# DigitalPhonetics/Intrinsic-Subgraph-Generation-for-VQA

Measured on AMD Instinct MI355X. Metric: GQA questions/sec, higher is better.
Workload: dtype f32

## Files before the change

### intrinsic-subgraph-generation-for-vqa_amd/csrc/isg_layer_tile.hip

```cpp
#include "isg_f16x3.hpp"

#include "isg_diag.hpp"

#include <type_traits>

ISG_DIAG_BUFFER(g_dt_stamps)
#define DT_STAMP(i) ISG_DIAG_ADD(i)
#define TC_STAMP(i) ISG_DIAG_ADD(i)

namespace isg {

constexpr int TP_CH = 1024;

__device__ __forceinline__ void tile_plan_body(const int *__restrict__ ptr, const int *__restrict__ eptr, int B, int ncap, int ecap,
                                               int *__restrict__ tile_ptr, int *__restrict__ ntiles, int cap,
                                               int4 *__restrict__ tile_info, int4 *__restrict__ tile_heavy_first = nullptr) {
  __shared__ int s_jump[2][TP_CH];
  __shared__ int s_mark[TP_CH];
  __shared__ int s_ptr[TP_CH + 1], s_eptr[TP_CH + 1];
  __shared__ int s_wsum[TP_CH / 64];
  __shared__ int s_base;
  const int i = threadIdx.x, lane = i & 63, wave = i >> 6;
  if (i == 0) s_base = 0;
  __syncthreads();
// ... 65 lines not shown
  if (tile_info && tile_heavy_first) {
    constexpr int NB = 9;
    constexpr int NW = TP_CH / 64;
    __shared__ int s_cnt[NW][NB];
    __shared__ int s_start[NB];
    __syncthreads();
    const int T = min(s_base, cap);
    int mine[NB];
#pragma unroll
    for (int b = 0; b < NB; ++b) mine[b] = 0;
    for (int t0 = 0; t0 < T; t0 += TP_CH) {
      const int t = t0 + i;
      const int cls = t < T ? NB - 1 - min((tile_info[t].w + 31) >> 5, NB - 1) : -1;
#pragma unroll
      for (int b = 0; b < NB; ++b) mine[b] += __popcll(__ballot(cls == b));
    }
    if (lane == 0) {
#pragma unroll
      for (int b = 0; b < NB; ++b) s_cnt[wave][b] = mine[b];
    }
    __syncthreads();
    if (i == 0) {
      int run = 0;
      for (int b = 0; b < NB; ++b) {
        int c = 0;
        for (int w = 0; w < NW; ++w) c += s_cnt[w][b];
        s_start[b] = run;
        run += c;
      }
    }
    __syncthreads();
    for (int t0 = 0; t0 < T; t0 += TP_CH) {
      const int t = t0 + i;
      int4 d = make_int4(0, 0, 0, 0);
      if (t < T) d = tile_info[t];
      const int cls = t < T ? NB - 1 - min((d.w + 31) >> 5, NB - 1) : -1;
      int below = 0, wcnt[NB];
#pragma unroll
      for (int b = 0; b < NB; ++b) {
        const unsigned long long m = __ballot(cls == b);
        wcnt[b] = __popcll(m);
        if (cls == b) below = __popcll(m & ((1ull << lane) - 1ull));
      }
      if (lane == 0) {
#pragma unroll
        for (int b = 0; b < NB; ++b) s_cnt[wave][b] = wcnt[b];
      }
      __syncthreads();
      if (cls >= 0) {
        int at = s_start[cls] + below;
        for (int w = 0; w < wave; ++w) at += s_cnt[w][cls];
        tile_heavy_first[at] = d;
      }
      __syncthreads();
      if (i < NB) {
        int c = 0;
        for (int w = 0; w < NW; ++w) c += s_cnt[w][i];
        s_start[i] += c;
      }
      __syncthreads();
    }
  }
}

__global__ __launch_bounds__(TP_CH) void tile_plan_kernel(const int *__restrict__ ptr, const int *__restrict__ eptr, int B,
                                                          int ncap, int ecap, int *__restrict__ tile_ptr,
                                                          int *__restrict__ ntiles, int cap, int4 *__restrict__ tile_info,
                                                          int4 *__restrict__ tile_heavy_first) {
  tile_plan_body(ptr, eptr, B, ncap, ecap, tile_ptr, ntiles, cap, tile_info, tile_heavy_first);
}

constexpr int DT_ROWS = 64, DT_KC = 128, DT_K1 = 512, DT_MID = 256, DT_C = 128;
constexpr int DT_LDA = DT_KC + 8, DT_LDY = DT_MID + 8, DT_LDC = DT_C + 4;
constexpr int DT_KS1 = DT_K1 / 16, DT_KS2 = DT_MID / 16;
constexpr int DT_BUF_BYTES = 2 * 2 * DT_ROWS * DT_LDA * 2;
constexpr int DT_GPC = 128;
constexpr int DT_GST = 8;
constexpr int DT_SMEM_BYTES = DT_BUF_BYTES + (3 * 64 + 4 * 64 + 64 + 64 + 64 + 2 * DT_GST * DT_C + DT_GPC + 4) * 4;
static_assert(2 * DT_ROWS * DT_LDY * 2 <= DT_BUF_BYTES && DT_ROWS * DT_LDC * 4 + 2 * 32 * DT_C * 4 <= DT_BUF_BYTES, "aliases must fit");
static_assert(2 * DT_SMEM_BYTES <= 160 * 1024, "two workgroups per CU");
constexpr int DT_GROUP_MAX = 4;
constexpr int DT_LIVE_SMEM_BYTES = DT_SMEM_BYTES + (DT_ROWS + DT_GROUP_MAX * DT_ROWS / 4 + 8) * 4;
static_assert(2 * DT_LIVE_SMEM_BYTES <= 160 * 1024, "two workgroups per CU");

struct DtArgs {
  const float *a;
  const float *a_rowmax;
  const _Float16 *w1f;
  const float *w1_inv, *b1;
  const float *y_bound;
  const _Float16 *w2f;
  const float *w2_inv, *b2;
  const float *ins, *h;
  const float *gn_w, *gn_b, *gn_ms;
  const float *node_mask, *ins_next;
  float *h_out;
  float *xg_out, *xinv_out;
  _Float16 *xp_out;
  const int *ptr, *tile_ptr, *ntiles;
  const int4 *tile_info;
  const long long *batch;
  int N, lda, P, ldp;
  float eps, denom;
  const unsigned *row_dead;
  int group, max_tiles;
};

template <bool LIVE>
__global__ __launch_bounds__(256, 2) void mgat_dense_tail_kernel(DtArgs a) {
  extern __shared__ __attribute__((aligned(16))) unsigned char dt_smem[];
  typedef _Float16 (*BufA)[2][DT_ROWS][DT_LDA];
  typedef _Float16 (*BufY)[DT_ROWS][DT_LDY];
  typedef float (*BufC)[DT_LDC];
  BufA bufA = reinterpret_cast<BufA>(dt_smem);
  BufY sY = reinterpret_cast<BufY>(dt_smem);
  BufC sC = reinterpret_cast<BufC>(dt_smem);
  float *s_f = reinterpret_cast<float *>(dt_smem + DT_BUF_BYTES);
  float *s_inv1 = s_f, *s_scale2 = s_f + 64, *s_inv2 = s_f + 128, *s_rmax = s_f + 192, *s_a = s_f + 448;
  int *s_gid = reinterpret_cast<int *>(s_f + 512);
  float *s_mask = s_f + 576;
  float *s_ins = s_f + 640, *s_insn = s_f + 640 + DT_GST * DT_C;

  int *s_gp = reinterpret_cast<int *>(s_f + 2688);
  int *s_list = reinterpret_cast<int *>(s_f + 2820);
  unsigned char *s_cpos = reinterpret_cast<unsigned char *>(s_f + 2884);
  int *s_w = reinterpret_cast<int *>(s_f + 2948);

  int tid = threadIdx.x, lane = tid & 63;
  const int wave = __builtin_amdgcn_readfirstlane(tid >> 6);
  int fr = lane & 31, hh = lane >> 5, fk = hh * 8;
  int srow = tid >> 5, sc4 = tid & 31;
  int gi = tid >> 5, c4 = tid & 31;
  int voff = lane * 16;
  int t = blockIdx.x, r0 = 0, nrows = 0, g0 = 0, g1 = 0, ng = 0, L = 0, tb = 0, t0 = 0, gt = 1;
  bool grouped = false;
  if constexpr (!LIVE) {
    const int4 tinfo = a.tile_info[t];
    if (t >= *a.ntiles) return;
    r0 = tinfo.x;
    nrows = min(tinfo.y, DT_ROWS);
    if (nrows <= 0) return;
    L = nrows;
    g0 = a.tile_ptr[t], g1 = a.tile_ptr[t + 1];
    ng = g1 - g0;
  } else {
    t0 = blockIdx.x * a.group;
    int4 ti[DT_GROUP_MAX];
#pragma unroll
    for (int k = 0; k < DT_GROUP_MAX; ++k) ti[k] = a.tile_info[min(t0 + k, a.max_tiles - 1)];
    const int nt = *a.ntiles;
    if (t0 >= nt) return;
    gt = min(a.group, nt - t0);
    int bk[DT_GROUP_MAX + 1];
    bk[0] = 0;
#pragma unroll
    for (int k = 0; k < DT_GROUP_MAX; ++k) bk[k + 1] = bk[k] + (k < gt ? max(min(ti[k].y, DT_ROWS), 0) : 0);
    const int total = bk[DT_GROUP_MAX];
    if (total == 0) return;
    int gr = ti[0].x + tid;
#pragma unroll
    for (int k = 1; k < DT_GROUP_MAX; ++k)
      if (tid >= bk[k]) gr = ti[k].x + tid - bk[k];
    const bool has = tid < total;
    gr = min(max(gr, 0), a.N - 1);
    const bool dead = has && a.row_dead[gr] == 0x01010101u;
    const bool live = has && !dead;
    const unsigned long long lb = __ballot(live), db = __ballot(dead);
    if (lane == 0) {
      s_w[wave] = __popcll(lb);
      s_w[4 + wave] = db ? wave * 64 + (int)__builtin_ctzll(db) : 256;
    }
    __syncthreads();
    int before = 0, nlive = 0, fd = 256;
#pragma unroll
    for (int w = 0; w < 4; ++w) {
      const int c = s_w[w];
      if (w < wave) before += c;
      nlive += c;
      fd = min(fd, s_w[4 + w]);
    }
    nlive = __builtin_amdgcn_readfirstlane(nlive);
    fd = __builtin_amdgcn_readfirstlane(fd);
    const int Lg = nlive + (fd < 256 ? 1 : 0);
    grouped = Lg <= DT_ROWS;
    if (grouped) {
      L = Lg;
      const int pos = before + __popcll(lb & ((1ull << lane) - 1ull));
      if (live) { s_list[pos] = gr; s_cpos[tid] = (unsigned char)pos; }
      if (dead) s_cpos[tid] = (unsigned char)nlive;
      if (tid == fd) s_list[nlive] = gr;
    }
  }
  ISG_DIAG_BEGIN()
  hf32x4 rh[8];
  int h_gid = 0, h_gp = 0;
  float h_mask = 1.f;
  float4 h_ins = make_float4(0.f, 0.f, 0.f, 0.f), h_insn = make_float4(0.f, 0.f, 0.f, 0.f);

#define DT_ROW(row) (LIVE ? s_list[min(row, L - 1)] : min(r0 + min(row, nrows - 1), a.N - 1))
  auto x_proj = [&](auto ni_c) __attribute__((always_inline)) {
  constexpr int NI = decltype(ni_c)::value;
  constexpr int NU = 4 * NI;
  if constexpr (LIVE) __syncthreads();
#define DT_LOAD_CHUNK(c)                                                                                         \
  _Pragma("unroll") for (int u = 0; u < NU; ++u) {                                                               \
    const int row = srow + 8 * u;                                                                                \
    const int gr = DT_ROW(row);                                                                                  \
    { const hf32x4 t_ = __builtin_nontemporal_load(reinterpret_cast<const hf32x4 *>(a.a + (int64_t)gr * a.lda + (c) * DT_KC + sc4 * 4)); ra[u] = make_float4(t_[0], t_[1], t_[2], t_[3]); } \
  }
  float4 ra[NU];
  DT_LOAD_CHUNK(0)
  const int hrow = DT_ROW(tid);
  const float *rm = a.a_rowmax + (int64_t)hrow * a.ldp;
  float rmv[4];
#pragma unroll
  for (int p = 0; p < 4; ++p) rmv[p] = rm[min(p, a.P - 1)];
#define DT_TAIL_REQUEST(trow)                                                                                    \
  h_gid = (int)a.batch[trow];                                                                                    \
  if (a.node_mask) h_mask = a.node_mask[trow];                       \
  h_gp = a.ptr[g0 + min(tid, ng)];                                                                               \
  {                                                                                                              \
    const int gi_c = min(gi, max(min(ng, DT_GST) - 1, 0));                                                       \
    h_ins = *reinterpret_cast<const float4 *>(a.ins + (int64_t)(g0 + gi_c) * DT_C + c4 * 4);                     \
    if (a.ins_next) h_insn = *reinterpret_cast<const float4 *>(a.ins_next + (int64_t)(g0 + gi_c) * DT_C + c4 * 4); \
  }
  if constexpr (!LIVE) { DT_TAIL_REQUEST(hrow) }
  if (tid < DT_ROWS) {
    float mx = fmaxf(fmaxf(rmv[0], rmv[1]), fmaxf(rmv[2], rmv[3]));
    for (int p = 4; p < a.P; ++p) mx = fmaxf(mx, rm[p]);
    float s, inv;
    h3_scale(mx, s, inv);
    s_rmax[tid] = s;
    s_inv1[tid] = inv;
    h3_scale(fmaf(mx, a.y_bound[0], a.y_bound[1]), s, inv);
    s_scale2[tid] = s;
    s_inv2[tid] = inv;
    if constexpr (!LIVE) {
      s_gid[tid] = h_gid;
      s_mask[tid] = h_mask;
    }
  }
#define DT_TAIL_FILE()                                                                                           \
  if (tid <= min(ng, DT_GPC)) s_gp[tid] = h_gp - r0;                                                             \
  if (gi < min(ng, DT_GST)) {                                                                                    \
    *reinterpret_cast<float4 *>(&s_ins[gi * DT_C + c4 * 4]) = h_ins;                                             \
    if (a.ins_next) *reinterpret_cast<float4 *>(&s_insn[gi * DT_C + c4 * 4]) = h_insn;                           \
  }
  if constexpr (!LIVE) { DT_TAIL_FILE() }
  __syncthreads();
  float sa[NU];
#pragma unroll
  for (int u = 0; u < NU; ++u) sa[u] = s_rmax[srow + 8 * u];
#define DT_WRITE_CHUNK(b)                                                                                        \
  _Pragma("unroll") for (int u = 0; u < NU; ++u) {                                                               \
    const int row = srow + 8 * u;                                                                                \
    float4 v = ra[u];                                                                                            \
    if (row >= L) v = make_float4(0.f, 0.f, 0.f, 0.f);                                                           \
    v.x *= sa[u]; v.y *= sa[u]; v.z *= sa[u]; v.w *= sa[u];                                                      \
    hf16x4 hi = {(_Float16)v.x, (_Float16)v.y, (_Float16)v.z, (_Float16)v.w};                                    \
    hf16x4 mid = {(_Float16)(v.x - (float)hi[0]), (_Float16)(v.y - (float)hi[1]), (_Float16)(v.z - (float)hi[2]), \
                  (_Float16)(v.w - (float)hi[3])};                                                               \
    *reinterpret_cast<hf16x4 *>(&bufA[b][0][row][sc4 * 4]) = hi;                                                 \
    *reinterpret_cast<hf16x4 *>(&bufA[b][1][row][sc4 * 4]) = mid;                                                \
  }
  DT_STAMP(0)
  DT_WRITE_CHUNK(0)
  DT_LOAD_CHUNK(1)

  constexpr unsigned plane1 = (unsigned)(DT_MID / 32) * DT_KS1 * 1024u;
  const __amdgpu_buffer_rsrc_t wr1 =
      __builtin_amdgcn_make_buffer_rsrc(const_cast<_Float16 *>(a.w1f), 0, (int)(2u * plane1), 0x00020000);
  hf32x16 acc[NI][2];
#pragma unroll
  for (int i = 0; i < NI; ++i)
#pragma unroll
    for (int j = 0; j < 2; ++j)
#pragma unroll
      for (int r = 0; r < 16; ++r) acc[i][j][r] = 0.f;
  hf16x8 wq[4][2][2], af[NI][2];
#define DT_LOADW1(st, s)                                                                                         \
  _Pragma("unroll") for (int j = 0; j < 2; ++j) _Pragma("unroll") for (int q = 0; q < 2; ++q)                    \
      wq[st][j][q] = __builtin_bit_cast(hf16x8, __builtin_amdgcn_raw_buffer_load_b128(                           \
          wr1, voff, (int)(((unsigned)(2 * wave + j) * DT_KS1 + (unsigned)(s)) * 1024u + q * plane1), 0));
#define DT_LOADA1(b, ksl)                                                                                        \
  _Pragma("unroll") for (int i = 0; i < NI; ++i) _Pragma("unroll") for (int q = 0; q < 2; ++q)                   \
      af[i][q] = *reinterpret_cast<const hf16x8 *>(&bufA[b][q][i * 32 + fr][(ksl) * 16 + fk]);
#define DT_MMA1(A, W)                                                                                            \
  _Pragma("unroll") for (int i = 0; i < NI; ++i) _Pragma("unroll") for (int j = 0; j < 2; ++j)                   \
      acc[i][j] = __builtin_amdgcn_mfma_f32_32x32x16_f16(W[j][1], A[i][0], acc[i][j], 0, 0, 0);                  \
  _Pragma("unroll") for (int i = 0; i < NI; ++i) _Pragma("unroll") for (int j = 0; j < 2; ++j)                   \
      acc[i][j] = __builtin_amdgcn_mfma_f32_32x32x16_f16(W[j][0], A[i][1], acc[i][j], 0, 0, 0);                  \
  _Pragma("unroll") for (int i = 0; i < NI; ++i) _Pragma("unroll") for (int j = 0; j < 2; ++j)                   \
      acc[i][j] = __builtin_amdgcn_mfma_f32_32x32x16_f16(W[j][0], A[i][0], acc[i][j], 0, 0, 0);
  DT_LOADW1(0, 0)
  DT_LOADW1(1, 1)
  DT_LOADW1(2, 2)
  __syncthreads();
  DT_STAMP(1)
#pragma unroll
  for (int s = 0; s < DT_KS1; ++s) {
    const int c = s >> 3, ksl = s & 7;
    if (s + 3 < DT_KS1) { DT_LOADW1((s + 3) & 3, s + 3) }
    DT_LOADA1(c & 1, ksl)
    __builtin_amdgcn_sched_barrier(0);
    DT_MMA1(af, wq[s & 3])
    __builtin_amdgcn_sched_barrier(0);
    if (ksl == 7 && c < 3) {
      DT_WRITE_CHUNK((c + 1) & 1)
      if (c + 2 < 4) { DT_LOAD_CHUNK(c + 2) }
      __syncthreads();
      DT_STAMP(2 + c)
    }
  }
  ISG_DIAG_KEEP2(acc[0][0][0], acc[NI - 1][1][15])
  DT_STAMP(5)
#undef DT_LOADW1
#undef DT_LOADA1
#undef DT_MMA1
#undef DT_LOAD_CHUNK
#undef DT_WRITE_CHUNK

  {
    hf32x4 wi4[2][4], bv4[2][4];
#pragma unroll
    for (int j = 0; j < 2; ++j)
#pragma unroll
      for (int g = 0; g < 4; ++g) {
        const int col = (2 * wave + j) * 32 + 8 * g + 4 * hh;
        wi4[j][g] = *reinterpret_cast<const hf32x4 *>(a.w1_inv + col);
        bv4[j][g] = *reinterpret_cast<const hf32x4 *>(a.b1 + col);
      }
// ... 153 lines not shown
  for (int gb = 0; gb < ng; gb += 32) {
    const int ge = min(ng, gb + 32);
    {
      const int ch = tid & (DT_C - 1);
      const float ms = a.gn_ms[ch];
      for (int gi = gb + (tid >> 7); gi < ge; gi += 2) {
        const int nb = gi < DT_GPC ? s_gp[gi] : a.ptr[g0 + gi] - r0;
        const int n = min(gi < DT_GPC ? s_gp[gi + 1] : a.ptr[g0 + gi + 1] - r0, nrows) - nb;
        if (n <= 0) continue;
        const float cnt = (float)n;
        float sum = 0.f;
#pragma unroll 4
        for (int k = 0; k < n; ++k) sum = add_rn(sum, mul_rn(s_a[nb + k], sC[crow(nb + k)][ch]));
        const float mean_ms = mul_rn(sum / cnt, ms);
        float sq = 0.f;
#pragma unroll 4
        for (int k = 0; k < n; ++k) {
          const float o = sub_rn(mul_rn(s_a[nb + k], sC[crow(nb + k)][ch]), mean_ms);
          sq = add_rn(sq, mul_rn(o, o));
        }
        s_mean[gi - gb][ch] = mean_ms;
        s_std[gi - gb][ch] = sqrtf(add_rn(sq / cnt, a.eps));
      }
    }
    __syncthreads();
    {
      const float4 w4 = *reinterpret_cast<const float4 *>(a.gn_w + sc4 * 4), b4 = *reinterpret_cast<const float4 *>(a.gn_b + sc4 * 4);
      const float wv[4] = {w4.x, w4.y, w4.z, w4.w}, bv[4] = {b4.x, b4.y, b4.z, b4.w};
#pragma unroll
      for (int u = 0; u < 8; ++u) {
        const int row = srow + 8 * u;
        const int gi = s_gid[min(row, nrows - 1)] - g0;
        if (row >= nrows || gi < gb || gi >= ge) continue;
        const float an = s_a[row], mk = s_mask[row];
        const float4 c4 = *reinterpret_cast<const float4 *>(&sC[crow(row)][sc4 * 4]);
        const float4 m4 = *reinterpret_cast<const float4 *>(&s_mean[gi - gb][sc4 * 4]);
        const float4 d4 = *reinterpret_cast<const float4 *>(&s_std[gi - gb][sc4 * 4]);
        float4 x4 = make_float4(0.f, 0.f, 0.f, 0.f);
        if (a.ins_next)
          x4 = gi < DT_GST ? *reinterpret_cast<const float4 *>(&s_insn[gi * DT_C + sc4 * 4])
                           : *reinterpret_cast<const float4 *>(a.ins_next + (int64_t)(g0 + gi) * DT_C + sc4 * 4);
        const float cv[4] = {c4.x, c4.y, c4.z, c4.w}, mv[4] = {m4.x, m4.y, m4.z, m4.w}, dv[4] = {d4.x, d4.y, d4.z, d4.w};
        const float xv[4] = {x4.x, x4.y, x4.z, x4.w};
        hf32x4 y4, g4;
#pragma unroll
        for (int j = 0; j < 4; ++j) {
          const float o = sub_rn(mul_rn(an, cv[j]), mv[j]);
          float y = add_rn(mul_rn(wv[j], o) / dv[j], bv[j]);
          y = add_rn(y, rh[u][j]);
          if (a.node_mask) y = mul_rn(mk, y);
          y4[j] = y;
        }
        if (a.xg_out || a.xp_out) {
          const isg_f32x2 ga = gelu_exact2(isg_f32x2{y4[0] * xv[0], y4[1] * xv[1]});
          const isg_f32x2 gb2 = gelu_exact2(isg_f32x2{y4[2] * xv[2], y4[3] * xv[3]});
          g4 = hf32x4{ga.x, ga.y, gb2.x, gb2.y};
        }
        const int64_t at = (int64_t)(r0 + row) * DT_C + sc4 * 4;
        *reinterpret_cast<hf32x4 *>(a.h_out + at) = y4;
        if (a.xg_out) *reinterpret_cast<hf32x4 *>(a.xg_out + at) = g4;
        if (a.xp_out) {
          const float mx = group_max<32>(fmaxf(fmaxf(fabsf(g4[0]), fabsf(g4[1])), fmaxf(fabsf(g4[2]), fabsf(g4[3]))));
          float sc, inv;
          h3_scale(mx, sc, inv);
          if (sc4 == 0) a.xinv_out[r0 + row] = inv;
          g4 *= sc;
          hf16x4 hi = {(_Float16)g4[0], (_Float16)g4[1], (_Float16)g4[2], (_Float16)g4[3]};
          hf16x4 mid = {(_Float16)(g4[0] - (float)hi[0]), (_Float16)(g4[1] - (float)hi[1]), (_Float16)(g4[2] - (float)hi[2]),
                        (_Float16)(g4[3] - (float)hi[3])};
          *reinterpret_cast<hf16x4 *>(a.xp_out + (int64_t)(r0 + row) * 256 + sc4 * 4) = hi;
          *reinterpret_cast<hf16x4 *>(a.xp_out + (int64_t)(r0 + row) * 256 + 128 + sc4 * 4) = mid;
        }
      }
    }
    if (gb + 32 < ng) __syncthreads();
  }
  DT_STAMP(11)
  };
#undef DT_ROW
#undef DT_TAIL_REQUEST
#undef DT_TAIL_FILE
#undef DT_LOAD_H

  if constexpr (!LIVE) {
    x_proj(std::integral_constant<int, 2>{});
    tail();
    ISG_DIAG_DUMP(g_dt_stamps, t * 4 + wave, 12, st_acc[13] = nrows; st_acc[14] = ng;)
  } else {
    bool have_c = false;
#pragma unroll 1
    for (int it = 0; it < gt; ++it) {
      asm volatile("" : "+v"(tid));
      lane = tid & 63, fr = lane & 31, hh = lane >> 5, fk = hh * 8, srow = tid >> 5, sc4 = tid & 31, gi = srow, c4 = sc4, voff = lane * 16;
      t = t0 + it;
      const int4 tinfo = a.tile_info[t];
      r0 = tinfo.x;
      nrows = min(tinfo.y, DT_ROWS);
      if (nrows <= 0) continue;
      g0 = a.tile_ptr[t], g1 = a.tile_ptr[t + 1];
      ng = g1 - g0;
      if (!grouped) {
        L = nrows;
        const int trow = min(r0 + min(tid, nrows - 1), a.N - 1);
        const bool dead = tid < nrows && a.row_dead[trow] == 0x01010101u;
        const unsigned long long db = __ballot(dead);
        if (tid < nrows) {
          s_list[tid] = dead ? min(r0 + (int)__builtin_ctzll(db), a.N - 1) : trow;
          s_cpos[tb + tid] = (unsigned char)tid;
        }
      }
      if (!grouped || !have_c) {
        if (L > 32) x_proj(std::integral_constant<int, 2>{}); else x_proj(std::integral_constant<int, 1>{});
        have_c = true;
      } else {
        __syncthreads();
      }
      tail();
      tb += nrows;
    }
    ISG_DIAG_DUMP(g_dt_stamps, blockIdx.x * 4 + wave, 12, st_acc[13] = L; st_acc[14] = gt;)
  }
}

}

using namespace isg;

ISG_DIAG_SETTER(isg_dt_set_stamp_buffer, g_dt_stamps)

extern "C" int64_t isg_tile_plan_capacity(int64_t N, int64_t E, int64_t B, int32_t node_cap, int32_t edge_cap) {
  if (N < 0 || E < 0 || B < 0 || node_cap <= 0) return 0;
  int64_t t = 2 * (N / node_cap + 1) + (B + TP_CH - 1) / TP_CH + 1;
  if (edge_cap > 0) t += 2 * (E / edge_cap + 1);
  return t < B ? t : B;
}

extern "C" int isg_tile_plan(const int32_t *ptr, const int32_t *eptr, int64_t B, int32_t node_cap, int32_t edge_cap,
                             int32_t *tile_ptr, int32_t *ntiles, int32_t *tile_info, int64_t capacity,
                             int32_t *tile_info_heavy_first, void *stream) {
  if (B < 0 || node_cap <= 0 || capacity < 0 || !tile_ptr || !ntiles || (B > 0 && !ptr) || (tile_info_heavy_first && !tile_info))
    return ISG_EINVAL;
  if (tile_info_heavy_first && (reinterpret_cast<uintptr_t>(tile_info_heavy_first) & 15) != 0) return ISG_EINVAL;
  if (eptr && edge_cap <= 0) return ISG_EINVAL;
  if (B >= (1ll << 31) || capacity >= (1ll << 31)) return ISG_EUNSUPPORTED;
  if (tile_info && (reinterpret_cast<uintptr_t>(tile_info) & 15) != 0) return ISG_EINVAL;
  tile_plan_kernel<<<1, TP_CH, 0, as_stream(stream)>>>(ptr, eptr, (int)B, node_cap, edge_cap, tile_ptr, ntiles, (int)capacity,
                                                       reinterpret_cast<int4 *>(tile_info),
                                                       reinterpret_cast<int4 *>(tile_info_heavy_first));
  return check_launch();
}

extern "C" int isg_mgat_dense_tail(const float *conv_out, int32_t lda, const float *a_rowmax, int32_t P, int32_t ldp,
                                   const uint16_t *w1_frag, const float *w1_inv_scale, const float *b1, const float *y_bound,
                                   const uint16_t *w2_frag, const float *w2_inv_scale, const float *b2, const float *ins,
                                   const float *h, const float *gn_weight, const float *gn_bias, const float *gn_mean_scale,
                                   double eps, const float *node_mask, const float *ins_next, float *h_out, float *xg_out,
                                   uint16_t *xp_out, float *xinv_out, const int32_t *ptr, const int64_t *batch,
                                   const int32_t *tile_ptr, const int32_t *tile_info, const int32_t *ntiles, int64_t max_tiles,
                                   const uint8_t *row_dead, int32_t group, int64_t N, int32_t K1, int32_t MID, int32_t C,
                                   void *stream) {
  if (N < 0 || max_tiles < 0 || lda < K1 || P <= 0 || ldp < P) return ISG_EINVAL;
  if (K1 != DT_K1 || MID != DT_MID || C != DT_C || (lda & 3) != 0 || N >= (1ll << 31) || max_tiles >= (1ll << 31) ||
      (reinterpret_cast<uintptr_t>(conv_out) & 15) != 0 || (reinterpret_cast<uintptr_t>(ins) & 15) != 0 ||
      ((reinterpret_cast<uintptr_t>(w1_inv_scale) | reinterpret_cast<uintptr_t>(b1) | reinterpret_cast<uintptr_t>(w2_inv_scale) |
        reinterpret_cast<uintptr_t>(b2)) & 15) != 0)
    return ISG_EUNSUPPORTED;
  if (N == 0 || max_tiles == 0) return ISG_OK;
  if (!conv_out || !a_rowmax || !w1_frag || !w1_inv_scale || !b1 || !y_bound || !w2_frag || !w2_inv_scale || !b2 || !ins || !h ||
      !gn_weight || !gn_bias || !gn_mean_scale || !h_out || !ptr || !batch || !tile_ptr || !tile_info || !ntiles ||
      ((xg_out || xp_out) && !ins_next) || (xp_out && !xinv_out))
    return ISG_EINVAL;
  static const bool dense_rows = [] { const char *e = getenv("ISG_DT_DENSE_ROWS"); return e && atoi(e) != 0; }();
  if (dense_rows) row_dead = nullptr;
  if (row_dead && (group < 1 || group > DT_GROUP_MAX || (reinterpret_cast<uintptr_t>(row_dead) & 3) != 0)) return ISG_EINVAL;
  if (!(row_dead ? dyn_lds_ok<&mgat_dense_tail_kernel<true>>(DT_LIVE_SMEM_BYTES) : dyn_lds_ok<&mgat_dense_tail_kernel<false>>(DT_SMEM_BYTES)))
    return ISG_EUNSUPPORTED;
  DtArgs a = {
      .a = conv_out, .a_rowmax = a_rowmax, .w1f = reinterpret_cast<const _Float16 *>(w1_frag), .w1_inv = w1_inv_scale, .b1 = b1,
      .y_bound = y_bound, .w2f = reinterpret_cast<const _Float16 *>(w2_frag), .w2_inv = w2_inv_scale, .b2 = b2, .ins = ins, .h = h,
      .gn_w = gn_weight, .gn_b = gn_bias, .gn_ms = gn_mean_scale, .node_mask = node_mask, .ins_next = ins_next, .h_out = h_out,
      .xg_out = xg_out, .xinv_out = xinv_out, .xp_out = reinterpret_cast<_Float16 *>(xp_out), .ptr = ptr, .tile_ptr = tile_ptr,
      .ntiles = ntiles, .tile_info = reinterpret_cast<const int4 *>(tile_info), .batch = reinterpret_cast<const long long *>(batch),
      .N = (int)N, .lda = lda, .P = P, .ldp = ldp, .eps = (float)eps, .denom = (float)sqrt((double)DT_C),
      .row_dead = reinterpret_cast<const unsigned *>(row_dead), .group = row_dead ? group : 1, .max_tiles = (int)max_tiles};
  if (!a.a || !a.a_rowmax || !a.w1f || !a.w1_inv || !a.b1 || !a.y_bound || !a.w2f || !a.w2_inv || !a.b2 || !a.ins || !a.h || !a.gn_w ||
      !a.gn_b || !a.gn_ms || !a.h_out || !a.ptr || !a.tile_ptr || !a.ntiles || !a.tile_info || !a.batch ||
      ((a.xg_out || a.xp_out) && !a.ins_next) || (a.xp_out && !a.xinv_out))
    return ISG_EINVAL;
  if (row_dead)
    mgat_dense_tail_kernel<true><<<(unsigned)((max_tiles + group - 1) / group), 256, DT_LIVE_SMEM_BYTES, as_stream(stream)>>>(a);
  else
    mgat_dense_tail_kernel<false><<<(unsigned)max_tiles, 256, DT_SMEM_BYTES, as_stream(stream)>>>(a);
  return check_launch();
}

namespace isg {

constexpr int TC_ROWS = 64, TC_ECAP = 256, TC_C = 128, TC_KC = 128, TC_LDX = TC_C + 4, TC_LDA = TC_KC + 8, TC_THREADS = 256;
constexpr int TC_SMEM_BYTES = TC_ROWS * TC_LDX * 4 + 2 * 64 * TC_LDA * 2 + TC_ECAP * 16 + TC_ECAP * 4 + 4 * 64 * 4 + 64 * 4 + 68 * 4 + 2 * TC_C * 4;
static_assert(2 * TC_SMEM_BYTES <= 160 * 1024, "two workgroups per CU");

struct TcArgs {
  const float *x_l, *x_r;
  const _Float16 *ep;
  const float *ep_inv;
  const _Float16 *Wf;
  const float *w_inv, *att;
  const float *bias;
  const int *rowptr, *eid, *src, *dst, *ntiles;
  const int4 *tile_info;
  const float *edge_mask, *node_mask;
  float *out, *alpha;
  float *rowmax;
  int N, E, H, K, KS, NT, ldl, ldr, ldo;
  float slope;
};

__device__ __forceinline__ void edge_planes_row(const float *__restrict__ edge_attr, int lda, const int *__restrict__ eid, int E, int K,
                                                _Float16 *__restrict__ planes, float *__restrict__ inv_out, int slot, int c4) {
  if (slot >= E) return;
  const unsigned e = eid ? (unsigned)eid[slot] : (unsigned)slot;
  float4 v = make_float4(0.f, 0.f, 0.f, 0.f);
  if (c4 * 4 < K && e < (unsigned)E) v = *reinterpret_cast<const float4 *>(edge_attr + (int64_t)e * lda + c4 * 4);
  const float mx = group_max<32>(fmaxf(fmaxf(fabsf(v.x), fabsf(v.y)), fmaxf(fabsf(v.z), fabsf(v.w))));
  float s, inv;
  h3_scale(mx, s, inv);
  if (c4 == 0) inv_out[slot] = inv;
  v.x *= s; v.y *= s; v.z *= s; v.w *= s;
  hf16x4 hi = {(_Float16)v.x, (_Float16)v.y, (_Float16)v.z, (_Float16)v.w};
  hf16x4 mid = {(_Float16)(v.x - (float)hi[0]), (_Float16)(v.y - (float)hi[1]), (_Float16)(v.z - (float)hi[2]),
                (_Float16)(v.w - (float)hi[3])};
  *reinterpret_cast<hf16x4 *>(planes + (int64_t)slot * 256 + c4 * 4) = hi;
  *reinterpret_cast<hf16x4 *>(planes + (int64_t)slot * 256 + 128 + c4 * 4) = mid;
}

__global__ __launch_bounds__(256) void edge_planes_kernel(const float *__restrict__ edge_attr, int lda, const int *__restrict__ eid,
                                                          int E, int K, _Float16 *__restrict__ planes, float *__restrict__ inv_out) {
  edge_planes_row(edge_attr, lda, eid, E, K, planes, inv_out, blockIdx.x * 8 + (threadIdx.x >> 5), threadIdx.x & 31);
}

__global__ __launch_bounds__(TP_CH) void tile_plan_edge_planes_kernel(const int *__restrict__ ptr, const int *__restrict__ eptr, int B,
                                                                      int ncap, int ecap, int *__restrict__ tile_ptr,
                                                                      int *__restrict__ ntiles, int cap, int4 *__restrict__ tile_info,
                                                                      int4 *__restrict__ tile_heavy_first,
                                                                      const float *__restrict__ edge_attr, int lda,
                                                                      const int *__restrict__ eid, int E, int K,
                                                                      _Float16 *__restrict__ planes, float *__restrict__ inv_out) {
  if (blockIdx.x == 0)
    tile_plan_body(ptr, eptr, B, ncap, ecap, tile_ptr, ntiles, cap, tile_info, tile_heavy_first);
  else
    edge_planes_row(edge_attr, lda, eid, E, K, planes, inv_out, (blockIdx.x - 1) * 32 + (threadIdx.x >> 5), threadIdx.x & 31);
}

template <bool MASKED>
__global__ __launch_bounds__(TC_THREADS, 2) void gatv2_tile_conv_kernel(TcArgs a) {
  extern __shared__ __attribute__((aligned(16))) unsigned char tc_smem[];
  typedef float (*BufX)[TC_LDX];
  typedef _Float16 (*BufP)[64][TC_LDA];
  BufX sXl = reinterpret_cast<BufX>(tc_smem);
  BufP sA = reinterpret_cast<BufP>(tc_smem + TC_ROWS * TC_LDX * 4);
  int4 *s_tab = reinterpret_cast<int4 *>(tc_smem + TC_ROWS * TC_LDX * 4 + 2 * 64 * TC_LDA * 2);
  float *s_lg = reinterpret_cast<float *>(s_tab + TC_ECAP);
  float *s_part = s_lg + TC_ECAP;
  float *s_inv = s_part + 4 * 64;
  int *s_rp = reinterpret_cast<int *>(s_inv + 64);
  float *s_att = reinterpret_cast<float *>(s_rp + 68), *s_winv = s_att + TC_C;

// ... 316 lines not shown
```

Before: 3.456 million.

## Process grouped dense-tail tiles with a single merged group tail

Adds a group-wide tail path for the LIVE dense-tail kernel. When several tiles are compacted into one workgroup, attention scores, per-graph softmax, graph-norm statistics and the output epilogue run once over the whole group instead of once per tile. Graph spans, dead-row bitmasks, masks and instruction rows are staged in shared memory, and h and ins_next rows are prefetched ahead. This path is on by default, and the previous per-tile tails can be restored with ISG_DT_TILE_TAILS. It is meant to cut repeated per-tile synchronisation and tail overhead, at the cost of more shared-memory bookkeeping, register pressure and more complex indexing.

```diff
diff --git a/intrinsic-subgraph-generation-for-vqa_amd/csrc/isg_layer_tile.hip b/intrinsic-subgraph-generation-for-vqa_amd/csrc/isg_layer_tile.hip
--- a/intrinsic-subgraph-generation-for-vqa_amd/csrc/isg_layer_tile.hip
+++ b/intrinsic-subgraph-generation-for-vqa_amd/csrc/isg_layer_tile.hip
@@ -171,6 +171,18 @@
 constexpr int DT_GROUP_MAX = 4;
 constexpr int DT_LIVE_SMEM_BYTES = DT_SMEM_BYTES + (DT_ROWS + DT_GROUP_MAX * DT_ROWS / 4 + 8) * 4;
 static_assert(2 * DT_LIVE_SMEM_BYTES <= 160 * 1024, "two workgroups per CU");
+constexpr int DT_GGST = 16;
+constexpr int DT_GSTAT = 20;
+constexpr int DT_GROUP_ROWS = DT_GROUP_MAX * DT_ROWS;
+static_assert(DT_GGST == 16, "the header requests the instruction rows in two rounds of eight");
+constexpr int DT_G_MASK = 256, DT_G_GID = 512, DT_G_INS = 640, DT_G_SPAN = 2688, DT_G_PROW = 2752, DT_G_DEAD = 2768, DT_G_TILE = 2776;
+static_assert(DT_G_MASK >= 192 + DT_ROWS && DT_G_MASK + DT_GROUP_ROWS <= DT_G_GID, "the masks start behind s_rmax's strip in use");
+static_assert(DT_G_GID + DT_GROUP_ROWS / 2 <= DT_G_INS && DT_G_INS + DT_GGST * DT_C <= DT_G_SPAN, "graph ids, instruction rows");
+static_assert(DT_G_SPAN + DT_GPC / 2 <= DT_G_PROW && DT_G_PROW + DT_ROWS / 4 <= DT_G_DEAD && DT_G_DEAD + 8 <= DT_G_TILE &&
+              DT_G_TILE + 4 * DT_GROUP_MAX <= 2820, "the group's small tables end before the row list");
+static_assert(DT_G_DEAD % 2 == 0 && DT_G_TILE % 4 == 0 && DT_BUF_BYTES % 16 == 0, "64-bit and 128-bit entries are aligned");
+static_assert(DT_ROWS * DT_LDC * 4 + 3 * DT_GSTAT * DT_C * 4 + DT_GROUP_ROWS * 4 <= DT_BUF_BYTES, "c, the statistics and a fit the staging region");
+static_assert(DT_GROUP_ROWS <= 256 && DT_ROWS <= 64, "a thread per row of the group; a graph's dead bits fit a 64-bit window");
 
 struct DtArgs {
   const float *a;
@@ -214,6 +226,14 @@
   int *s_list = reinterpret_cast<int *>(s_f + 2820);
   unsigned char *s_cpos = reinterpret_cast<unsigned char *>(s_f + 2884);
   int *s_w = reinterpret_cast<int *>(s_f + 2948);
+  float *g_mask = s_f + DT_G_MASK, *g_ins = s_f + DT_G_INS;
+  unsigned short *g_gid = reinterpret_cast<unsigned short *>(s_f + DT_G_GID), *g_span = reinterpret_cast<unsigned short *>(s_f + DT_G_SPAN);
+  unsigned char *g_prow = reinterpret_cast<unsigned char *>(s_f + DT_G_PROW);
+  unsigned long long *g_dead = reinterpret_cast<unsigned long long *>(s_f + DT_G_DEAD);
+  int4 *g_tile = reinterpret_cast<int4 *>(s_f + DT_G_TILE);
+  float(*g_mean)[DT_C] = reinterpret_cast<float(*)[DT_C]>(dt_smem + DT_ROWS * DT_LDC * 4);
+  float(*g_std)[DT_C] = g_mean + DT_GSTAT, (*g_dvec)[DT_C] = g_mean + 2 * DT_GSTAT;
+  float *g_a = &g_mean[3 * DT_GSTAT][0];
 
   int tid = threadIdx.x, lane = tid & 63;
   const int wave = __builtin_amdgcn_readfirstlane(tid >> 6);
@@ -223,6 +243,11 @@
   int voff = lane * 16;
   int t = blockIdx.x, r0 = 0, nrows = 0, g0 = 0, g1 = 0, ng = 0, L = 0, tb = 0, t0 = 0, gt = 1;
   bool grouped = false;
+  bool gtail = false;
+  int nlive_g = 0, G0 = 0, NG = 0, total_g = 0;
+  int q_gid = 0, q_p0 = 0, q_p1 = 0, q_r0 = 0, q_bk = 0, q_nr = 0;
+  float q_mask = 1.f;
+  float4 q_ins0 = make_float4(0.f, 0.f, 0.f, 0.f), q_ins1 = q_ins0;
   if constexpr (!LIVE) {
     const int4 tinfo = a.tile_info[t];
     if (t >= *a.ntiles) return;
@@ -233,13 +258,17 @@
     g0 = a.tile_ptr[t], g1 = a.tile_ptr[t + 1];
     ng = g1 - g0;
   } else {
-    t0 = blockIdx.x * a.group;
+    const int G = a.group < 0 ? -a.group : a.group;
+    t0 = blockIdx.x * G;
     int4 ti[DT_GROUP_MAX];
+    int tp[DT_GROUP_MAX + 1];
 #pragma unroll
     for (int k = 0; k < DT_GROUP_MAX; ++k) ti[k] = a.tile_info[min(t0 + k, a.max_tiles - 1)];
+#pragma unroll
+    for (int k = 0; k <= DT_GROUP_MAX; ++k) tp[k] = a.tile_ptr[min(t0 + k, a.max_tiles)];
     const int nt = *a.ntiles;
     if (t0 >= nt) return;
-    gt = min(a.group, nt - t0);
+    gt = min(G, nt - t0);
     int bk[DT_GROUP_MAX + 1];
     bk[0] = 0;
 #pragma unroll
@@ -254,6 +283,24 @@
     gr = min(max(gr, 0), a.N - 1);
     const bool dead = has && a.row_dead[gr] == 0x01010101u;
     const bool live = has && !dead;
+    if (a.group > 0) {
+      G0 = tp[0];
+      NG = tp[1] - G0;
+#pragma unroll
+      for (int k = 2; k <= DT_GROUP_MAX; ++k)
+        if (k == gt) NG = tp[k] - G0;
+      q_gid = (int)a.batch[gr];
+      if (a.node_mask) q_mask = a.node_mask[gr];
+      q_r0 = ti[0].x, q_bk = 0, q_nr = bk[1];
+#pragma unroll
+      for (int k = 1; k < DT_GROUP_MAX; ++k)
+        if (k < gt && G0 + tid >= tp[k]) q_r0 = ti[k].x, q_bk = bk[k], q_nr = bk[k + 1] - bk[k];
+      q_p0 = a.ptr[G0 + min(tid, NG)];
+      q_p1 = a.ptr[G0 + min(tid + 1, NG)];
+      const int gq_last = max(min(NG, DT_GGST) - 1, 0);
+      q_ins0 = *reinterpret_cast<const float4 *>(a.ins + (int64_t)(G0 + min(gi, gq_last)) * DT_C + c4 * 4);
+      q_ins1 = *reinterpret_cast<const float4 *>(a.ins + (int64_t)(G0 + min(gi + 8, gq_last)) * DT_C + c4 * 4);
+    }
     const unsigned long long lb = __ballot(live), db = __ballot(dead);
     if (lane == 0) {
       s_w[wave] = __popcll(lb);
@@ -278,6 +325,15 @@
       if (live) { s_list[pos] = gr; s_cpos[tid] = (unsigned char)pos; }
       if (dead) s_cpos[tid] = (unsigned char)nlive;
       if (tid == fd) s_list[nlive] = gr;
+      gtail = a.group > 0;
+      if (gtail) {
+        nlive_g = nlive, total_g = total;
+        if (live) g_prow[pos] = (unsigned char)tid;
+        if (lane == 0) g_dead[wave] = db;
+#pragma unroll
+        for (int k = 0; k < DT_GROUP_MAX; ++k)
+          if (tid == k && k < gt) g_tile[k] = make_int4(ti[k].x, bk[k + 1] - bk[k], bk[k], tp[k] - G0);
+      }
     }
   }
   ISG_DIAG_BEGIN()
@@ -336,6 +392,20 @@
     if (a.ins_next) *reinterpret_cast<float4 *>(&s_insn[gi * DT_C + c4 * 4]) = h_insn;                           \
   }
   if constexpr (!LIVE) { DT_TAIL_FILE() }
+  if constexpr (LIVE) {
+    if (gtail) {
+      if (tid < total_g) {
+        g_gid[tid] = (unsigned short)(q_gid - G0);
+        g_mask[tid] = q_mask;
+      }
+      if (tid < min(NG, DT_GPC)) {
+        const int nb = q_p0 - q_r0, n = min(q_p1 - q_r0, q_nr) - nb;
+        g_span[tid] = n > 0 ? (unsigned short)((q_bk + nb) | (n << 8)) : (unsigned short)0;
+      }
+      if (gi < min(NG, DT_GGST)) *reinterpret_cast<float4 *>(&g_ins[gi * DT_C + c4 * 4]) = q_ins0;
+      if (gi + 8 < min(NG, DT_GGST)) *reinterpret_cast<float4 *>(&g_ins[(gi + 8) * DT_C + c4 * 4]) = q_ins1;
+    }
+  }
   __syncthreads();
   float sa[NU];
 #pragma unroll
@@ -655,6 +725,241 @@
 #undef DT_TAIL_FILE
 #undef DT_LOAD_H
 
+  auto group_tail = [&]() __attribute__((always_inline)) {
+  if constexpr (LIVE) {
+    typedef unsigned long long u64;
+    const int nlive = nlive_g, crep = min(nlive, L - 1);
+    auto span = [&](int gg, int &nb, int &n) __attribute__((always_inline)) {
+      if (gg < DT_GPC) {
+        const int s = g_span[gg];
+        nb = s & 255, n = s >> 8;
+        return;
+      }
+      int k = 0;
+      for (int j = 1; j < gt; ++j)
+        if (g_tile[j].w <= gg) k = j;
+      const int4 tl = g_tile[k];
+      const int p0 = a.ptr[G0 + gg] - tl.x, p1 = a.ptr[G0 + gg + 1] - tl.x;
+      n = min(p1, tl.y) - p0, nb = tl.z + p0;
+      if (n <= 0) nb = 0, n = 0;
+    };
+    auto dead_win = [&](int nb, int n) __attribute__((always_inline)) -> u64 {
+      const int q = nb >> 6, s = nb & 63;
+      u64 w = g_dead[q] >> s;
+      if (s != 0 && q < DT_GROUP_ROWS / 64 - 1) w |= g_dead[q + 1] << (64 - s);
+      return n >= 64 ? w : w & ((1ull << n) - 1ull);
+    };
+    constexpr int DT_PRE = 2;
+    hf32x4 rhg[DT_PRE][8], xh[8];
+#pragma unroll
+    for (int u = 0; u < 8; ++u) xh[u] = hf32x4{0.f, 0.f, 0.f, 0.f};
+    auto load_h = [&](int k, int u) __attribute__((always_inline)) -> hf32x4 {
+      const int4 tl = g_tile[k];
+      const int gr = min(tl.x + min(srow + 8 * u, tl.y - 1), a.N - 1);
+      return __builtin_nontemporal_load(reinterpret_cast<const hf32x4 *>(a.h + (int64_t)gr * DT_C + sc4 * 4));
+    };
+    auto load_front = [&]() __attribute__((always_inline)) {
+#pragma unroll
+      for (int k = 0; k < DT_PRE; ++k) {
+        if (k < gt && g_tile[k].y > 0) {
+#pragma unroll
+          for (int u = 0; u < 8; ++u) rhg[k][u] = load_h(k, u);
+        }
+      }
+    };
+    load_front();
+    auto load_x = [&](int k, int u) __attribute__((always_inline)) {
+      const int4 tl = g_tile[k];
+      const int row = min(srow + 8 * u, tl.y - 1);
+      if (a.ins_next) xh[u] = *reinterpret_cast<const hf32x4 *>(a.ins_next + (int64_t)(G0 + (int)g_gid[tl.z + row]) * DT_C + sc4 * 4);
+    };
+    int first = 0;
+    while (first < gt - 1 && g_tile[first].y <= 0) ++first;
+#pragma unroll
+    for (int u = 0; u < 8; ++u) load_x(first, u);
+
+    const int NE = nlive + NG;
+    for (int eb = 8 * wave; eb < NE; eb += 32) {
+      float part[4];
+      int wr[4];
+#pragma unroll
+      for (int u = 0; u < 4; ++u) {
+        const int e = eb + 2 * u + hh;
+        int gg, cr, row = -1;
+        if (e < nlive) {
+          row = g_prow[e];
+          gg = g_gid[row];
+          cr = e;
+        } else {
+          gg = min(e - nlive, NG - 1);
+          cr = crep;
+          int nb, n;
+          span(gg, nb, n);
+          if (e < NE && n > 0) {
+            const u64 w = dead_win(nb, n);
+            if (w) row = nb + (int)__builtin_ctzll(w);
+          }
+        }
+        const float4 q = gg < DT_GGST ? *reinterpret_cast<const float4 *>(&g_ins[gg * DT_C + fr * 4])
+                                      : *reinterpret_cast<const float4 *>(a.ins + (int64_t)(G0 + gg) * DT_C + fr * 4);
+        const float4 v = *reinterpret_cast<const float4 *>(&sC[cr][fr * 4]);
+        part[u] = 0.f + dot4_rn(v, q);
+        wr[u] = row;
+      }
+#pragma unroll
+      for (int u = 0; u < 4; ++u) part[u] = group_sum<32>(part[u]);
+#pragma unroll
+      for (int u = 0; u < 4; ++u)
+        if (fr == 0 && wr[u] >= 0) g_a[wr[u]] = part[u] / a.denom;
+    }
+    __syncthreads();
+    DT_STAMP(9)
+    for (int gg = wave; gg < NG; gg += 4) {
+      int nb, n;
+      span(gg, nb, n);
+      nb = __builtin_amdgcn_readfirstlane(nb), n = __builtin_amdgcn_readfirstlane(n);
+      if (n <= 0) continue;
+      const u64 w = dead_win(nb, n);
+      float *sa_g = g_a + nb;
+      const int src = ((w >> lane) & 1) ? (int)__builtin_ctzll(w) : lane;
+      const float v = lane < n ? sa_g[src] : -INFINITY;
+      const float mx = wave_max(v);
+      __builtin_amdgcn_wave_barrier();
+      if (lane < n) sa_g[lane] = expf(v - mx);
+      __builtin_amdgcn_wave_barrier();
+      float sum = 0.f;
+      for (int k = 0; k < n; ++k) sum += sa_g[k];
+      sum += 0.f;
+      __builtin_amdgcn_wave_barrier();
+      if (lane < n) sa_g[lane] = sa_g[lane] / sum;
+    }
+    __syncthreads();
+    DT_STAMP(10)
+    for (int gb = 0; gb < NG; gb += DT_GSTAT) {
+      const int ge = min(NG, gb + DT_GSTAT);
+      if (gb > 0) {
+        load_front();
+#pragma unroll
+        for (int u = 0; u < 8; ++u) load_x(first, u);
+      }
+      {
+        const int ch = tid & (DT_C - 1);
+        const float ms = a.gn_ms[ch], gw = a.gn_w[ch], gbias = a.gn_b[ch];
+        for (int gg = gb + (tid >> 7); gg < ge; gg += 2) {
+          int nb, n;
+          span(gg, nb, n);
+          nb = __builtin_amdgcn_readfirstlane(nb), n = __builtin_amdgcn_readfirstlane(n);
+          if (n <= 0) continue;
+          const u64 wv_ = dead_win(nb, n);
+          const u64 w = ((u64)(unsigned)__builtin_amdgcn_readfirstlane((int)(wv_ >> 32)) << 32) |
+                        (u64)(unsigned)__builtin_amdgcn_readfirstlane((int)wv_);
+          const float cnt = (float)n;
+          float v_dead = 0.f;
+          if (w) v_dead = mul_rn(g_a[nb + (int)__builtin_ctzll(w)], sC[crep][ch]);
+          const u64 lbits = ~w & (n >= 64 ? ~0ull : (1ull << n) - 1ull);
+          auto in_order = [&](float dead_term, auto live_term) __attribute__((always_inline)) -> float {
+            float acc = 0.f;
+            u64 lw = lbits;
+            for (int k = 0; k < n;) {
+              const int j = lw ? (int)__builtin_ctzll(lw) : n;
+              float av = 0.f, cv = 0.f;
+              if (j < n) av = g_a[nb + j], cv = sC[s_cpos[nb + j]][ch];
+              int r = j - k;
+              for (; r >= 4; r -= 4) acc = add_rn(add_rn(add_rn(add_rn(acc, dead_term), dead_term), dead_term), dead_term);
+              if (r & 2) acc = add_rn(add_rn(acc, dead_term), dead_term);
+              if (r & 1) acc = add_rn(acc, dead_term);
+              if (j < n) acc = add_rn(acc, live_term(av, cv));
+              lw &= lw - 1ull;
+              k = j + 1;
+            }
+            return acc;
+          };
+          const float sum = in_order(v_dead, [&](float av, float cv) { return mul_rn(av, cv); });
+          const float mean_ms = mul_rn(sum / cnt, ms);
+          const float o_dead = sub_rn(v_dead, mean_ms), oo_dead = mul_rn(o_dead, o_dead);
+          const float sq = in_order(oo_dead, [&](float av, float cv) {
+            const float o = sub_rn(mul_rn(av, cv), mean_ms);
+            return mul_rn(o, o);
+          });
+          const float sd = sqrtf(add_rn(sq / cnt, a.eps));
+          g_mean[gg - gb][ch] = mean_ms;
+          g_std[gg - gb][ch] = sd;
+          if (w) g_dvec[gg - gb][ch] = add_rn(mul_rn(gw, o_dead) / sd, gbias);
+        }
+      }
+      __syncthreads();
+      DT_STAMP(11)
+      {
+        const float4 w4 = *reinterpret_cast<const float4 *>(a.gn_w + sc4 * 4), b4 = *reinterpret_cast<const float4 *>(a.gn_b + sc4 * 4);
+        const float wv[4] = {w4.x, w4.y, w4.z, w4.w}, bv[4] = {b4.x, b4.y, b4.z, b4.w};
+#pragma unroll
+        for (int it = 0; it < DT_GROUP_MAX; ++it) {
+          if (it >= gt) break;
+          const int4 tl = g_tile[it];
+          const bool later = it + DT_PRE < gt && g_tile[min(it + DT_PRE, DT_GROUP_MAX - 1)].y > 0;
+          int nx = it + 1;
+          while (nx < gt && g_tile[nx].y <= 0) ++nx;
+#pragma unroll
+          for (int u = 0; u < 8; ++u) {
+            const int row = srow + 8 * u;
+            const hf32x4 hrow = rhg[it % DT_PRE][u], xrow = xh[u];
+            if (later) rhg[it % DT_PRE][u] = load_h(it + DT_PRE, u);
+            if (tl.y <= 0) continue;
+            if (nx < gt) load_x(nx, u);
+            const int grow = tl.z + min(row, tl.y - 1);
+            const int gg = g_gid[grow];
+            if (row >= tl.y || gg < gb || gg >= ge) continue;
+            const bool isdead = (g_dead[grow >> 6] >> (grow & 63)) & 1;
+            const float mk = g_mask[grow];
+            float yv[4];
+            if (isdead) {
+              const float4 d4 = *reinterpret_cast<const float4 *>(&g_dvec[gg - gb][sc4 * 4]);
+              yv[0] = d4.x, yv[1] = d4.y, yv[2] = d4.z, yv[3] = d4.w;
+            } else {
+              const float an = g_a[grow];
+              const float4 c4 = *reinterpret_cast<const float4 *>(&sC[s_cpos[grow]][sc4 * 4]);
+              const float4 m4 = *reinterpret_cast<const float4 *>(&g_mean[gg - gb][sc4 * 4]);
+              const float4 d4 = *reinterpret_cast<const float4 *>(&g_std[gg - gb][sc4 * 4]);
+              const float cv[4] = {c4.x, c4.y, c4.z, c4.w}, mv[4] = {m4.x, m4.y, m4.z, m4.w}, dv[4] = {d4.x, d4.y, d4.z, d4.w};
+#pragma unroll
+              for (int j = 0; j < 4; ++j) yv[j] = add_rn(mul_rn(wv[j], sub_rn(mul_rn(an, cv[j]), mv[j])) / dv[j], bv[j]);
+            }
+            hf32x4 y4, g4;
+#pragma unroll
+            for (int j = 0; j < 4; ++j) {
+              float y = add_rn(yv[j], hrow[j]);
+              if (a.node_mask) y = mul_rn(mk, y);
+              y4[j] = y;
+            }
+            if (a.xg_out || a.xp_out) {
+              const isg_f32x2 ga = gelu_exact2(isg_f32x2{y4[0] * xrow[0], y4[1] * xrow[1]});
+              const isg_f32x2 gb2 = gelu_exact2(isg_f32x2{y4[2] * xrow[2], y4[3] * xrow[3]});
+              g4 = hf32x4{ga.x, ga.y, gb2.x, gb2.y};
+            }
+            const int64_t at = (int64_t)(tl.x + row) * DT_C + sc4 * 4;
+            *reinterpret_cast<hf32x4 *>(a.h_out + at) = y4;
+            if (a.xg_out) *reinterpret_cast<hf32x4 *>(a.xg_out + at) = g4;
+            if (a.xp_out) {
+              const float mx = group_max<32>(fmaxf(fmaxf(fabsf(g4[0]), fabsf(g4[1])), fmaxf(fabsf(g4[2]), fabsf(g4[3]))));
+              float sc, inv;
+              h3_scale(mx, sc, inv);
+              if (sc4 == 0) a.xinv_out[tl.x + row] = inv;
+              g4 *= sc;
+              hf16x4 hi = {(_Float16)g4[0], (_Float16)g4[1], (_Float16)g4[2], (_Float16)g4[3]};
+              hf16x4 mid = {(_Float16)(g4[0] - (float)hi[0]), (_Float16)(g4[1] - (float)hi[1]), (_Float16)(g4[2] - (float)hi[2]),
+                            (_Float16)(g4[3] - (float)hi[3])};
+              *reinterpret_cast<hf16x4 *>(a.xp_out + (int64_t)(tl.x + row) * 256 + sc4 * 4) = hi;
+              *reinterpret_cast<hf16x4 *>(a.xp_out + (int64_t)(tl.x + row) * 256 + 128 + sc4 * 4) = mid;
+            }
+          }
+        }
+      }
+      DT_STAMP(15)
+      if (ge < NG) __syncthreads();
+    }
+  }
+  };
+
   if constexpr (!LIVE) {
     x_proj(std::integral_constant<int, 2>{});
     tail();
@@ -688,6 +993,12 @@
       } else {
         __syncthreads();
       }
+      if (gtail) {
+        asm volatile("" : "+v"(tid));
+        lane = tid & 63, fr = lane & 31, hh = lane >> 5, srow = tid >> 5, sc4 = tid & 31;
+        group_tail();
+        break;
+      }
       tail();
       tb += nrows;
     }
@@ -745,6 +1056,7 @@
     return ISG_EINVAL;
   static const bool dense_rows = [] { const char *e = getenv("ISG_DT_DENSE_ROWS"); return e && atoi(e) != 0; }();
   if (dense_rows) row_dead = nullptr;
+  static const bool tile_tails = [] { const char *e = getenv("ISG_DT_TILE_TAILS"); return e && atoi(e) != 0; }();
   if (row_dead && (group < 1 || group > DT_GROUP_MAX || (reinterpret_cast<uintptr_t>(row_dead) & 3) != 0)) return ISG_EINVAL;
   if (!(row_dead ? dyn_lds_ok<&mgat_dense_tail_kernel<true>>(DT_LIVE_SMEM_BYTES) : dyn_lds_ok<&mgat_dense_tail_kernel<false>>(DT_SMEM_BYTES)))
     return ISG_EUNSUPPORTED;
@@ -755,7 +1067,7 @@
       .xg_out = xg_out, .xinv_out = xinv_out, .xp_out = reinterpret_cast<_Float16 *>(xp_out), .ptr = ptr, .tile_ptr = tile_ptr,
       .ntiles = ntiles, .tile_info = reinterpret_cast<const int4 *>(tile_info), .batch = reinterpret_cast<const long long *>(batch),
       .N = (int)N, .lda = lda, .P = P, .ldp = ldp, .eps = (float)eps, .denom = (float)sqrt((double)DT_C),
-      .row_dead = reinterpret_cast<const unsigned *>(row_dead), .group = row_dead ? group : 1, .max_tiles = (int)max_tiles};
+      .row_dead = reinterpret_cast<const unsigned *>(row_dead), .group = row_dead ? (tile_tails ? -group : group) : 1, .max_tiles = (int)max_tiles};
   if (!a.a || !a.a_rowmax || !a.w1f || !a.w1_inv || !a.b1 || !a.y_bound || !a.w2f || !a.w2_inv || !a.b2 || !a.ins || !a.h || !a.gn_w ||
       !a.gn_b || !a.gn_ms || !a.h_out || !a.ptr || !a.tile_ptr || !a.ntiles || !a.tile_info || !a.batch ||
       ((a.xg_out || a.xp_out) && !a.ins_next) || (a.xp_out && !a.xinv_out))
```

Result: no change. 3.475 million, median of 6 (+0.6%).
